# NVlabs/motion-policy-networks

Hardware: AMD Instinct MI355X
Metric: env-steps/sec (FK+SDF+PointNet++) (higher is better)
Workload: dtype f32

## Files before the change

include/mpinets_hip.h:

```cpp
#ifndef MPINETS_HIP_H
#define MPINETS_HIP_H

#include <stdint.h>

#ifdef __cplusplus
extern "C" {
#endif

typedef void *mpx_stream_t;

#define MPX_NUM_FRAMES 15

int mpx_version(void);
const char *mpx_last_error(void);
int mpx_device_info(char *name, int name_len, int *cu_count, int *lds_bytes);


int mpx_prim_frames(const float *centers, const float *quats, int n, float *inv_frames,
                    mpx_stream_t stream);

int mpx_cuboid_sdf(const float *inv_frames, const float *dims, int B, int M, const float *points,
                   int P, float *out, mpx_stream_t stream);
int mpx_cylinder_sdf(const float *inv_frames, const float *radii, const float *heights, int B,
                     int M, const float *points, int P, float *out, mpx_stream_t stream);
// ... 137 lines not shown

int mpx_scene_cloud(const float *cub_centers, const float *cub_dims, const float *cub_quats, int M1,
                    const float *cyl_centers, const float *cyl_radii, const float *cyl_heights,
                    const float *cyl_quats, int M2, int B, int num_points, uint64_t seed,
                    int64_t env_offset, uint16_t *assign, uint8_t *labels, int32_t *n_obstacles, float *out,
                    int64_t out_batch_stride, int out_point_stride, int write_label,
                    mpx_stream_t stream);


int mpx_fps(const float *xyz, int B, int N, int stride, int npoint, int32_t *idx, float *new_xyz,
            int new_stride, mpx_stream_t stream);

#define MPX_VARIANT_FPS 0
#define MPX_VARIANT_BALL_QUERY 1
#define MPX_VARIANT_UNIT_QUEUE 2
#define MPX_VARIANT_COUNT_ 3
int mpx_set_variant(int what, int value);
int mpx_get_variant(int what);

int mpx_ball_query(const float *new_xyz, int new_stride, const float *xyz, int stride, int B,
                   int N, int npoint, float radius, int nsample, int32_t *idx, int32_t *cnt,
                   mpx_stream_t stream);

int mpx_ball_query_hits(const float *new_xyz, int new_stride, const float *xyz, int stride, int B,
                        int N, int npoint, float radius, int nsample, int32_t *idx, int32_t *cnt,
                        mpx_stream_t stream);

int mpx_sort_queries(const int32_t *cnt, int64_t n, int nsample, int32_t *order, int32_t *scratch,
                     mpx_stream_t stream);

int mpx_group_points(const float *xyz, int stride, const float *new_xyz, int new_stride,
                     const float *feat, int feat_stride, int C, const int32_t *idx, int B, int N,
                     int npoint, int nsample, float *out, mpx_stream_t stream);

int mpx_sa_mlp(const float *xyz, int stride, const float *new_xyz, int new_stride,
               const float *feat, int feat_stride, int C, const int32_t *idx, const int32_t *cnt,
               int B, int N, int npoint, int nsample, const float *wpack, int c1, int c2, int c3,
               float *out, int out_stride, int append_centre, mpx_stream_t stream);
int mpx_sa_mlp_factored(const float *pre, const float *ctr, const int32_t *idx, const int32_t *cnt, int B,
                        int N, int npoint, int nsample, const float *wpack, int C, int c1, int c2, int c3,
                        float *out, int out_stride, mpx_stream_t stream);
int mpx_sa_mlp_bf16x3_factored_wants_order(void);
int mpx_sa_mlp_bf16x3_factored(const float *pre, const float *ctr, const int32_t *idx, const int32_t *cnt,
                               const int32_t *order, int B, int N, int npoint, int nsample, const void *wpack,
                               int C, int c1, int c2, int c3, float *out, int out_stride, mpx_stream_t stream);
int64_t mpx_sa_pack_size(int C, int c1, int c2, int c3);
int mpx_sa_pack_weights(const float *w1, const float *b1, const float *w2, const float *b2,
                        const float *w3, const float *b3, int C, int c1, int c2, int c3,
                        float *wpack, mpx_stream_t stream);

int mpx_sa_mlp_bf16x3_wants_order(int C, int c1, int c2, int c3, int nsample);
int mpx_sa_mlp_bf16x3(const float *xyz, int stride, const float *new_xyz, int new_stride,
                      const float *feat, int feat_stride, int C, const int32_t *idx,
                      const int32_t *cnt, const int32_t *order, int B, int N, int npoint,
                      int nsample, const void *wpack, int c1, int c2, int c3, float *out,
                      int out_stride, int append_centre, mpx_stream_t stream);
// ... 106 lines not shown
```

motion-policy-networks_amd/csrc/common.h:

```cpp
#pragma once
#include <hip/hip_runtime.h>

#include <atomic>
#include <type_traits>
#include <stdint.h>
#include <stdio.h>

#include "../../include/mpinets_hip.h"

#define MPX_EXPORT extern "C" __attribute__((visibility("default")))

void mpx_set_error(const char *fmt, ...);

#define MPX_REQUIRE(cond, ...)        \
  do {                                \
    if (!(cond)) {                    \
      mpx_set_error(__VA_ARGS__);     \
      return 1;                       \
    }                                 \
  } while (0)

#define MPX_LDS_LIMIT_ONCE(kernel, bytes, what)                                                                \
  do {                                                                                                         \
    static std::atomic<unsigned long long> lds_done_{0};                                                       \
// ... 10 lines not shown

#define MPX_LAUNCH_CHECK(name)                                              \
  do {                                                                      \
    hipError_t e_ = hipGetLastError();                                      \
    if (e_ != hipSuccess) {                                                 \
      mpx_set_error("%s: launch failed: %s", name, hipGetErrorString(e_)); \
      return 2;                                                             \
    }                                                                       \
    return 0;                                                               \
  } while (0)

static inline hipStream_t mpx_s(mpx_stream_t s) { return reinterpret_cast<hipStream_t>(s); }
unsigned int *mpx_unit_queue_for(hipStream_t stream, int *exhausted);
int mpx_unit_queue_slots();
void mpx_unit_queue_set_slots(int n);
static inline int cdiv(int64_t a, int64_t b) { return (int)((a + b - 1) / b); }

int mpx_segmax_check(const char *name, int M, const int32_t *seg, int64_t Q, int N, const void *keys, const float *pooled,
                     int ldp, const int64_t *arg);
int mpx_segmax_unpack_launch(const unsigned long long *keys, int64_t Q, int N, float *pooled, int ldp, int64_t *arg,
                             hipStream_t stream);
void mpx_wgrad_bf16x3_launch(const float *dy, int lddy, const float *x, int ldx, int M, int N, int K, int rows_per_split,
                             int S, float *partial, int with_bias, hipStream_t stream);
void mpx_reduce_partials_launch(const float *partial, int S, int64_t stride, int64_t n, float *out, hipStream_t stream);

constexpr int MPX_GRID_Y = 65535;
static inline int64_t mpx_row_slab(int bm, int64_t row_bytes) {
  int64_t blocks = 65528;
  if (row_bytes > 0) {
    const int64_t fit = ((((int64_t)1 << 32) - 8192) / row_bytes / bm) & ~(int64_t)7;
// ... 206 lines not shown
```

motion-policy-networks_amd/csrc/pointnet.hip:

```cpp
#include "common.h"

#include <stdlib.h>
#include <type_traits>

typedef unsigned long long u64;

template <int CTRL>
__device__ __forceinline__ u64 dpp_mov64(u64 v) {
  unsigned lo = (unsigned)v, hi = (unsigned)(v >> 32);
  lo = (unsigned)__builtin_amdgcn_update_dpp(0, (int)lo, CTRL, 0xf, 0xf, true);
  hi = (unsigned)__builtin_amdgcn_update_dpp(0, (int)hi, CTRL, 0xf, 0xf, true);
  return ((u64)hi << 32) | lo;
}
struct U32Pair {
  unsigned lo, hi;
};
__device__ __forceinline__ u64 pack64(unsigned lo, unsigned hi) { return __builtin_bit_cast(u64, U32Pair{lo, hi}); }
__device__ __forceinline__ u64 umax64(u64 a, u64 b) {
  double r;
  asm("v_max_f64 %0, %1, %2" : "=v"(r) : "v"(__builtin_bit_cast(double, a)), "v"(__builtin_bit_cast(double, b)));
  return __builtin_bit_cast(u64, r);
}

__device__ __forceinline__ u64 row_max64(u64 v) {
// ... 509 lines not shown
  }
}

#ifndef MPX_FPS4_MIN_B
#define MPX_FPS4_MIN_B 768
#endif
constexpr int FPS_MAX_N = 8192;
constexpr int FPS_MAX_LDS = 256 + 3 * FPS_MAX_N * 4;

static int opt_n_threads_log2(int n) {
  int l = 0;
  while ((2 << l) <= n && (2 << l) <= 512) ++l;
  return l;
}

static std::atomic<int> g_variant[MPX_VARIANT_COUNT_] = {{1}, {1}, {1}};
MPX_EXPORT int mpx_set_variant(int what, int value) {
  MPX_REQUIRE(what >= 0 && what < MPX_VARIANT_COUNT_, "mpx_set_variant: unknown selector %d", what);
  MPX_REQUIRE(value == 0 || value == 1, "mpx_set_variant: value must be 0 (plain kernels) or 1 (default)");
  g_variant[what].store(value, std::memory_order_relaxed);
  if (what == MPX_VARIANT_UNIT_QUEUE) mpx_unit_queue_set_slots(value ? 256 : 0);
  return 0;
}
MPX_EXPORT int mpx_get_variant(int what) {
  return (what >= 0 && what < MPX_VARIANT_COUNT_) ? g_variant[what].load(std::memory_order_relaxed) : -1;
}

MPX_EXPORT int mpx_fps(const float *xyz, int B, int N, int stride, int npoint, int32_t *idx, float *new_xyz,
                       int new_stride, mpx_stream_t stream) {
  MPX_REQUIRE(B >= 0 && N >= 1 && npoint >= 0 && stride >= 3, "mpx_fps: bad size");
  MPX_REQUIRE(N <= FPS_MAX_N, "mpx_fps: N = %d > %d unsupported", N, FPS_MAX_N);
// ... 627 lines not shown
```

motion-policy-networks_amd/csrc/sa_mlp.hip:

```cpp
#include "common.h"

#include <stdlib.h>
#include <type_traits>

typedef float f32x16 __attribute__((ext_vector_type(16)));

#define PAD_CH (-1)
constexpr int SA_MAX_NSAMPLE = 256;
#ifndef MPX_SA1_Q
#define MPX_SA1_Q 32
#endif
#ifndef MPX_SA2_Q
#define MPX_SA2_Q 8
#endif
#ifndef MPX_SA1_GR
#define MPX_SA1_GR 2
#endif
#ifndef MPX_SA_SPREAD
#define MPX_SA_SPREAD 1
#endif
#ifndef MPX_SA1_LDSPOOL
#define MPX_SA1_LDSPOOL 1
#endif

template <int CF, int C1, int C2, int C3>
struct SaCfg {
  static_assert(CF == 1 || CF % 2 == 0, "feature channels must be 1 or even");
  static_assert(C1 % 32 == 0 && C2 % 32 == 0 && C3 % 32 == 0, "layer widths must be multiples of 32");
  static constexpr int CIN = 3 + CF;
  static constexpr int KS0 = (CF == 1) ? 2 : 2 + CF / 2;
  static constexpr int KS1 = C1 / 2, KS2 = C2 / 2;
  static constexpr int OT1 = C1 / 32, OT2 = C2 / 32, OT3 = C3 / 32;
// ... 202 lines not shown
    }
  }

  float *orow = out + qid * out_stride;
#pragma unroll
  for (int ot = 0; ot < Cfg::OT3; ++ot) {
    float v = omax[ot];
    v = mpx_max_across_halves(v);
    const int ch = ot * 32 + col;
    v = fmaxf(v + bias3[ch], 0.0f);
    if (half == 0) orow[ch] = v;
  }
}


template <int CF, int C1, int C2, int C3, int Q, bool FACT, int MAXNS = SA_MAX_NSAMPLE>
__global__ void __launch_bounds__(64) __attribute__((amdgpu_waves_per_eu(CF == 1 ? 4 : 2, CF == 1 ? 4 : 2)))
    sa_mlp_packed_kernel(const float *__restrict__ xyz, int stride, const float *__restrict__ new_xyz,
                         int new_stride, const float *__restrict__ feat, int feat_stride,
                         const int32_t *__restrict__ idx, const int32_t *__restrict__ cnt, int64_t n_query, int N,
                         int npoint, int nsample, const float *__restrict__ wpack, float *__restrict__ out,
                         int out_stride, int bpe, const float *__restrict__ pre_rows, const float *__restrict__ ctr,
                         int append_centre, unsigned int *__restrict__ queue) {
  using Cfg = SaCfg<CF, C1, C2, C3>;
  constexpr int GR = CF == 1 ? MPX_SA1_GR : 4, NGRP = 32 / GR;
  static_assert(GR == 2 || GR == 4, "pooling groups of 2 or 4 rows");
  __shared__ float ctr_s[FACT ? Q * C1 : 1];
  constexpr bool LPOOL = CF == 1 && !FACT && MPX_SA1_LDSPOOL != 0 && MAXNS <= 128;
  __shared__ __attribute__((aligned(16))) float pool_s[LPOOL ? Q * C3 : 1];
  __shared__ __attribute__((aligned(16))) unsigned char qmap_s[Q * MAXNS / GR + 32];
  __shared__ __attribute__((aligned(16))) float b1_s[C1], b2_s[C2], b3_s[C3];
  static_assert(Q >= 1 && Q <= 32, "queries per wave");
  const int lane = threadIdx.x & 63;
  const int half = lane >> 5, col = lane & 31;
  const int64_t n_units = (n_query + Q - 1) / Q;
  const int xcd = blockIdx.x & 7;
  const int64_t j_end = bpe > 0 ? n_units / 8 : n_units;
  int steal = 0;
  auto next_unit = [&]() __attribute__((always_inline)) {
    unsigned int v = 0;
    if (lane == 0) v = atomicAdd(queue + (bpe > 0 ? ((xcd + steal) & 7) : 0), 1u);
    return (int64_t)(unsigned int)__builtin_amdgcn_readfirstlane((int)v);
  };
  const __amdgpu_buffer_rsrc_t wrsrc =
      __builtin_amdgcn_make_buffer_rsrc(const_cast<float *>(wpack), 0, (int)(Cfg::TOTAL * 4), 0x00020000);
  const int wvoff = lane * 16;
  for (int i = threadIdx.x; i < C1; i += 64) b1_s[i] = wpack[Cfg::B1_OFF + i];
  for (int i = threadIdx.x; i < C2; i += 64) b2_s[i] = wpack[Cfg::B2_OFF + i];
  for (int i = threadIdx.x; i < C3; i += 64) b3_s[i] = wpack[Cfg::B3_OFF + i];
  constexpr int G1 = FACT ? 0 : Cfg::S1 / 4, G2 = Cfg::S2 / 4, G3 = Cfg::S3 / 4, GT = G1 + G2 + G3;
  constexpr bool LAZY = FACT && MPX_SA_SPREAD;
  constexpr int CH = 4, NC0 = (GT + CH - 1) / CH, NC = NC0 + (NC0 & 1);
// ... 8 lines not shown
    int wb = (int)(FACT ? Cfg::W2_OFF : Cfg::W1_OFF) * 4;
    asm volatile("" : "+s"(wb));
    fetch(0, wb);
  }
  int64_t j_next = queue ? next_unit() : 0;
  for (bool first = true;; first = false) {
  int64_t wg;
  if (queue) {
    int64_t j = j_next;
    bool dry = false;
    while (j >= j_end) {
      if (bpe == 0 || ++steal == 8) {
        dry = true;
        break;
      }
      j = next_unit();
    }
    if (dry) break;
    wg = bpe > 0 ? ((j / bpe) * 8 + ((xcd + steal) & 7)) * bpe + j % bpe : j;
  } else {
    if (!first) break;
    wg = blockIdx.x;
    if (bpe > 0) {
      const int64_t slot = wg >> 3;
      wg = ((slot / bpe) * 8 + xcd) * bpe + slot % bpe;
    }
  }
  const int64_t q0 = wg * Q;
  const int nq = (int)min((int64_t)Q, n_query - q0);
  if constexpr (LPOOL) {
    const float ninf = -__builtin_inff();
#pragma unroll
    for (int e = lane; e < Q * C3 / 4; e += 64) *reinterpret_cast<float4 *>(pool_s + 4 * e) = make_float4(ninf, ninf, ninf, ninf);
  }
  if constexpr (FACT) {
#pragma unroll
    for (int i = threadIdx.x; i < Q * C1 / 4; i += 64) {
      const int qi = (4 * i) / C1;
      if (qi < nq)
        *reinterpret_cast<float4 *>(ctr_s + 4 * i) = *reinterpret_cast<const float4 *>(ctr + q0 * C1 + 4 * i);
    }
    __syncthreads();
  }

  int my_cnt = 0, my_rows = 0;
  if (lane < nq) {
    const int c = cnt[q0 + lane];
    my_cnt = c <= 0 ? 1 : (c > nsample ? nsample : c);
// ... 296 lines not shown
            __builtin_amdgcn_sched_group_barrier(0x020, 1, 0);
          }
        } else {
#pragma unroll
          for (int u = 0; u < CH; ++u) {
            __builtin_amdgcn_sched_group_barrier(0x008, 4, 0);
            __builtin_amdgcn_sched_group_barrier(0x020, 1, 0);
          }
        }
      }
    }
    if constexpr (!LPOOL) cur = gq(NGRP - 1);
  }
  if constexpr (LPOOL) {
#pragma unroll 2
    for (int e = lane; e < Q * C3 / 4; e += 64) {
      const int qi = (4 * e) / C3, ch = (4 * e) % C3;
      if (qi < nq) {
        const float4 v = *reinterpret_cast<const float4 *>(pool_s + 4 * e), bb = *reinterpret_cast<const float4 *>(b3_s + ch);
        *reinterpret_cast<float4 *>(out + (int64_t)(qbase + qi) * out_stride + ch) =
            make_float4(fmaxf(v.x + bb.x, 0.0f), fmaxf(v.y + bb.y, 0.0f), fmaxf(v.z + bb.z, 0.0f), fmaxf(v.w + bb.w, 0.0f));
      }
    }
  } else {
#pragma unroll
    for (int ot = 0; ot < Cfg::OT3; ++ot) flush(ot, cur);
  }
  }
}

static int64_t sa_wave_slots(int per_cu) {
  static std::atomic<int> cus[64];
  int dev = 0;
  if (hipGetDevice(&dev) != hipSuccess) return 0;
  int n = cus[dev & 63].load(std::memory_order_relaxed);
  if (n == 0) {
    if (hipDeviceGetAttribute(&n, hipDeviceAttributeMultiprocessorCount, dev) != hipSuccess || n <= 0) return 0;
    cus[dev & 63].store(n, std::memory_order_relaxed);
  }
  return ((int64_t)n * per_cu) & ~(int64_t)7;
}
template <int CF, int C1, int C2, int C3>
static int launch_sa(const float *xyz, int stride, const float *new_xyz, int new_stride, const float *feat,
                     int feat_stride, const int32_t *idx, const int32_t *cnt, int B, int N, int npoint, int nsample,
                     const float *wpack, float *out, int out_stride, int append_centre, mpx_stream_t stream) {
  const int64_t nq = (int64_t)B * npoint;
  MPX_REQUIRE(nq / 4 + 1 < ((int64_t)1 << 31), "mpx_sa_mlp: too many query points");
  MPX_REQUIRE(!append_centre || (cnt && out_stride >= C3 + 4),
              "mpx_sa_mlp: append_centre needs the hit counts and out_stride >= c3 + 4");
  MPX_REQUIRE(!append_centre || nsample <= SA_MAX_NSAMPLE, "mpx_sa_mlp: append_centre needs nsample <= %d", SA_MAX_NSAMPLE);
  if (cnt && nsample <= SA_MAX_NSAMPLE) {
    constexpr int QL = CF == 1 ? MPX_SA1_Q : 8, QS = CF == 1 ? 4 : 2;
    int rc = 0;
    auto go = [&](auto qtag) {
      constexpr int Q = decltype(qtag)::value;
      int64_t nw = (nq + Q - 1) / Q;
// ... 1 lines not shown
      unsigned int *queue = nullptr;
      const int64_t slots = sa_wave_slots(CF == 1 ? 16 : 8);
      if (slots > 0 && nw >= 4 * slots) {
        int exhausted = 0;
        queue = mpx_unit_queue_for(mpx_s(stream), &exhausted);
        if (!queue && !exhausted) {
          mpx_set_error("mpx_sa_mlp: cannot reset the unit queue");
          rc = 1;
          return;
        }
        if (queue) nw = slots;
      }
      bool lpool = false;
      if constexpr (CF == 1 && MPX_SA1_LDSPOOL != 0) {
        lpool = nsample <= 128 && out_stride % 4 == 0 && ((uintptr_t)out & 15) == 0;
        if (lpool)
          hipLaunchKernelGGL((sa_mlp_packed_kernel<CF, C1, C2, C3, Q, false, 128>), dim3((unsigned)nw), dim3(64), 0,
                             mpx_s(stream), xyz, stride, new_xyz, new_stride, feat, feat_stride, idx, cnt, nq, N, npoint,
                             nsample, wpack, out, out_stride, bpe, nullptr, nullptr, append_centre, queue);
      }
      if (!lpool)
        hipLaunchKernelGGL((sa_mlp_packed_kernel<CF, C1, C2, C3, Q, false>), dim3((unsigned)nw), dim3(64), 0,
                           mpx_s(stream), xyz, stride, new_xyz, new_stride, feat, feat_stride, idx, cnt, nq, N, npoint,
                           nsample, wpack, out, out_stride, bpe, nullptr, nullptr, append_centre, queue);
    };
    if (nq >= 1024 * QL) go(std::integral_constant<int, QL>{});
    else go(std::integral_constant<int, QS>{});
    if (rc) return rc;
  } else {
    hipLaunchKernelGGL((sa_mlp_kernel<CF, C1, C2, C3>), dim3((unsigned)((nq + 3) / 4)), dim3(256), 0,
// ... 47 lines not shown
    constexpr int Q = decltype(qtag)::value;
    int64_t nw = (nq + Q - 1) / Q;
    const int bpe = (npoint % Q == 0 && B % 8 == 0) ? npoint / Q : 0;
    unsigned int *queue = nullptr;
    const int64_t slots = sa_wave_slots(8);
    if (slots > 0 && nw >= 4 * slots) {
      int exhausted = 0;
      queue = mpx_unit_queue_for(mpx_s(stream), &exhausted);
      if (!queue && !exhausted) {
        mpx_set_error("mpx_sa_mlp_factored: cannot reset the unit queue");
        rc = 1;
        return;
      }
      if (queue) nw = slots;
    }
    hipLaunchKernelGGL((sa_mlp_packed_kernel<64, 128, 128, 256, Q, true>), dim3((unsigned)nw), dim3(64), 0,
                       mpx_s(stream), nullptr, 0, nullptr, 0, nullptr, 0, idx, cnt, nq, N, npoint, nsample, wpack, out,
                       out_stride, bpe, pre, ctr, 0, queue);
  };
  if (nq >= 1024 * MPX_SA2_Q) go(std::integral_constant<int, MPX_SA2_Q>{});
  else if (nq >= 1024) go(std::integral_constant<int, 2>{});
  else go(std::integral_constant<int, 1>{});
  if (rc) return rc;
  MPX_LAUNCH_CHECK("mpx_sa_mlp_factored");
}

MPX_EXPORT int64_t mpx_sa_pack_size(int C, int c1, int c2, int c3) {
#define CALL(a, b, c, d) return SaCfg<a, b, c, d>::TOTAL
  if (C == 1 && c1 == 64 && c2 == 64 && c3 == 64) { CALL(1, 64, 64, 64); }
  else if (C == 64 && c1 == 128 && c2 == 128 && c3 == 256) { CALL(64, 128, 128, 256); }
// ... 21 lines not shown
```

motion-policy-networks_amd/mpinets_amd/_lib.py:

```python
from __future__ import annotations

import ctypes
import os
from ctypes import c_char_p, c_float, c_int, c_int64, c_void_p
from typing import Optional

import torch

_HERE = os.path.dirname(os.path.abspath(__file__))
LIB_PATH = os.environ.get("MPX_LIB_PATH") or os.path.join(_HERE, "libmpinets_hip.so")

P, I, F, L = c_void_p, c_int, c_float, c_int64

PROTOTYPES = {
    "mpx_version": [],
    "mpx_device_info": [c_char_p, I, P, P],
    "mpx_prim_frames": [P, P, I, P, P],
    "mpx_cuboid_sdf": [P, P, I, I, P, I, P, P],
    "mpx_cylinder_sdf": [P, P, P, I, I, P, I, P, P],
    "mpx_sphere_sdf": [P, P, I, I, P, I, P, P],
    "mpx_franka_fk": [P, I, F, P, P],
    "mpx_franka_cloud": [P, I, F, P, P, P, I, P, L, I, P],
    "mpx_pose_cloud": [P, I, P, P, I, P, L, I, P],
    "mpx_franka_spheres": [P, I, F, P, P, I, P, P],
# ... 19 lines not shown
    "mpx_pool_dgrad": [P, I, P, P, I, P, L, I, I, P, I, P, I, I, I, I, P, I, P],
    "mpx_batch_configs": [P, L, I, P, P, P, F, ctypes.c_uint64, L, I, I, F, P, P, P, P, P, P],
    "mpx_gather_rows": [P, P, I, I, P, P],
    "mpx_depth_render": [P, F, F, F, F, I, I, I, P, P, I, P, P, P, I, P, P, I, F, P, P],
    "mpx_depth_select": [P, P, F, F, F, F, I, I, I, I, ctypes.c_uint64, L, P, L, I, P, P],
    "mpx_scene_cloud": [P, P, P, I, P, P, P, P, I, I, I, ctypes.c_uint64, L, P, P, P, P, L, I, I, P],
    "mpx_set_variant": [I, I],
    "mpx_get_variant": [I],
    "mpx_fps": [P, I, I, I, I, P, P, I, P],
    "mpx_ball_query": [P, I, P, I, I, I, I, F, I, P, P, P],
    "mpx_ball_query_hits": [P, I, P, I, I, I, I, F, I, P, P, P],
    "mpx_sort_queries": [P, L, I, P, P, P],
    "mpx_group_points": [P, I, P, I, P, I, I, P, I, I, I, I, P, P],
    "mpx_sa_mlp": [P, I, P, I, P, I, I, P, P, I, I, I, I, P, I, I, I, P, I, I, P],
    "mpx_sa_mlp_factored": [P, P, P, P, I, I, I, I, P, I, I, I, I, P, I, P],
    "mpx_sa_mlp_bf16x3_factored_wants_order": [],
    "mpx_sa_mlp_bf16x3_factored": [P, P, P, P, P, I, I, I, I, P, I, I, I, I, P, I, P],
    "mpx_sa_pack_size": [I, I, I, I],
    "mpx_sa_pack_weights": [P, P, P, P, P, P, I, I, I, I, P, P],
    "mpx_sa_mlp_bf16x3": [P, I, P, I, P, I, I, P, P, P, I, I, I, I, P, I, I, I, P, I, I, P],
    "mpx_sa_mlp_bf16x3_wants_order": [I, I, I, I, I],
    "mpx_sa_pack_bf16x3_size": [I, I, I, I],
    "mpx_sa_pack_bf16x3": [P, P, P, P, P, P, I, I, I, I, P, P],
    "mpx_sa3_pack_size": [I, I, I, I],
    "mpx_sa3_pack_weights": [P, I, P, P, P, P, P, I, I, I, I, P, P],
    "mpx_sa3_chain": [P, I, I, I, P, I, I, I, I, P, I, P],
    "mpx_sa3_chain_probe": [P, I, I, P, P, I, P, P],
    "mpx_sa2_bf16x3_set_probe": [P],
    "mpx_linear": [P, I, P, P, I, I, I, I, P, I, P],
    "mpx_linear_workspace": [I, I, I],
# ... 15 lines not shown
    "mpx_linear_dact": [P, I, P, I, I, I, P, I, I, P, I, P],
    "mpx_linear_bf16x3_dact": [P, I, P, I, I, I, P, I, I, P, I, P],
    "mpx_linear_wgrad_bf16x3": [P, I, P, I, I, I, I, P, P, P, P],
    "mpx_linear_wgrad_scratch": [I, I, I],
    "mpx_linear_wgrad": [P, I, P, I, I, I, I, P, P, P, P],
    "mpx_groupnorm_leaky": [P, P, P, I, I, I, F, P, P],
    "mpx_groupnorm_leaky_to_pairs": [P, P, P, I, I, I, F, P, I, P],
    "mpx_rowmax": [P, I, I, I, I, P, I, P],
    "mpx_append_columns": [P, I, I, I, L, P, I, I, P],
    "mpx_policy_workspace": [I, I],
    "mpx_policy_forward": [P, P, I, P, I, P, P, L, P],
    "mpx_rollout_workspace": [I, I],
    "mpx_rollout_step": [P, P, P, I, P, P, I, P, P, P, L, P],
    "mpx_rollout": [P, P, P, P, I, P, P, I, P, P, P, L, P],
}
RESTYPES = {"mpx_last_error": c_char_p, "mpx_sa_pack_size": c_int64, "mpx_sa3_front_bf16x3_pack_size": c_int64, "mpx_sa_pack_bf16x3_size": c_int64,
            "mpx_linear_wgrad_scratch": c_int64, "mpx_pool_wgrad_scratch": c_int64, "mpx_linear_workspace": c_int64, "mpx_policy_workspace": c_int64, "mpx_rollout_workspace": c_int64}

_lib: Optional[ctypes.CDLL] = None


class MpxError(RuntimeError):
    pass


def load() -> ctypes.CDLL:
    global _lib
    if _lib is not None:
        return _lib
    if not os.path.exists(LIB_PATH):
        raise MpxError(
# ... 93 lines not shown
```

motion-policy-networks_amd/mpinets_amd/pointnet2.py:

```python
from __future__ import annotations

from typing import Any, Callable, List, Optional, Tuple

import torch
from torch import nn

from . import _lib


def furthest_point_sample(xyz: torch.Tensor, npoint: int, return_xyz: bool = False):
    _lib.require_cuda(xyz)
    assert xyz.ndim == 3 and xyz.size(2) >= 3 and xyz.dtype == torch.float32 and xyz.is_contiguous()
    B, N, S = xyz.shape
    idx = torch.empty((B, npoint), dtype=torch.int32, device=xyz.device)
    new_xyz = torch.empty((B, npoint, 3), dtype=torch.float32, device=xyz.device) if return_xyz else None
    _lib.call("mpx_fps", _lib.ptr(xyz), B, N, S, npoint, _lib.ptr(idx), _lib.ptr(new_xyz), 3)
    return (idx, new_xyz) if return_xyz else idx


def gather_operation(features: torch.Tensor, idx: torch.Tensor) -> torch.Tensor:
    return torch.gather(features, 2, idx.long().unsqueeze(1).expand(-1, features.size(1), -1))


def ball_query(radius: float, nsample: int, xyz: torch.Tensor, new_xyz: torch.Tensor, return_counts: bool = False):
# ... 32 lines not shown
    need = _lib.load().mpx_linear_workspace(M, N, K)
    if need == 0:
        _lib.call("mpx_linear", _lib.ptr(x), x.stride(0), _lib.ptr(weight), _lib.ptr(bias), M, N, K, act,
                  _lib.ptr(out), out.stride(0))
    else:
        key = (x.device, _lib.stream_ptr())
        ws = _WORKSPACE.get(key)
        if ws is None or ws.numel() < need:
            ws = _WORKSPACE[key] = torch.empty(max(need, 16 << 20), dtype=torch.uint8, device=x.device)
        _lib.call("mpx_linear_ws", _lib.ptr(x), x.stride(0), _lib.ptr(weight), _lib.ptr(bias), M, N, K, act,
                  _lib.ptr(out), out.stride(0), _lib.ptr(ws), ws.numel())
    return out


_WORKSPACE = {}


def split_pairs(x: torch.Tensor, out: Optional[torch.Tensor] = None) -> torch.Tensor:
    assert x.ndim == 2 and x.stride(1) == 1 and x.dtype == torch.float32
    R, K = x.shape
    Kp = (K + 15) // 16 * 16
    if out is None:
        out = torch.empty((R, 2 * Kp), dtype=torch.bfloat16, device=x.device)
    assert out.shape == (R, 2 * Kp) and out.stride(1) == 1
    _lib.call("mpx_split_bf16", _lib.ptr(x), x.stride(0), R, K, _lib.ptr(out), out.stride(0))
    return out


class DerivedWeights:

# ... 86 lines not shown
                raise _lib.MpxError(f"unsupported shared-MLP shape C={C} mlp=({c1},{c2},{c3})")
            _lib.call(fn, _lib.ptr(w[0]), _lib.ptr(b[0]), _lib.ptr(w[1]), _lib.ptr(b[1]), _lib.ptr(w[2]),
                      _lib.ptr(b[2]), C, c1, c2, c3, _lib.ptr(pack))
            return pack

        return self.entry(("pack", precision), [p for c in convs for p in (c.weight, c.bias)], make)


def launch_sa(precision: str, xyz_ptr: int, stride: int, new_xyz_ptr: int, new_stride: int, feat_ptr: int,
              feat_stride: int, C: int, idx: torch.Tensor, cnt: Optional[torch.Tensor], B: int, N: int, npoint: int,
              nsample: int, wpack: torch.Tensor, widths: Tuple[int, int, int], out_ptr: int, out_stride: int,
              append_centre: bool = False) -> bool:
    c1, c2, c3 = widths
    if precision == "fp32":
        fused = bool(append_centre and cnt is not None)
        _lib.call("mpx_sa_mlp", xyz_ptr, stride, new_xyz_ptr, new_stride, feat_ptr, feat_stride, C, _lib.ptr(idx),
                  _lib.ptr(cnt), B, N, npoint, nsample, _lib.ptr(wpack), c1, c2, c3, out_ptr, out_stride, int(fused))
        return fused
    order = None
    wants_order = bool(_lib.load().mpx_sa_mlp_bf16x3_wants_order(C, c1, c2, c3, nsample))
    if cnt is not None and wants_order:
        order = torch.empty(B * npoint, dtype=torch.int32, device=idx.device)
        scratch = torch.empty(128, dtype=torch.int32, device=idx.device)
        _lib.call("mpx_sort_queries", _lib.ptr(cnt), B * npoint, nsample, _lib.ptr(order), _lib.ptr(scratch))
    fused = bool(append_centre and not wants_order)
    _lib.call("mpx_sa_mlp_bf16x3", xyz_ptr, stride, new_xyz_ptr, new_stride, feat_ptr, feat_stride, C, _lib.ptr(idx),
              _lib.ptr(cnt), _lib.ptr(order), B, N, npoint, nsample, _lib.ptr(wpack), c1, c2, c3, out_ptr, out_stride,
              int(fused))
    return fused

# ... 11 lines not shown
    launch_sa(precision, _lib.ptr(xyz), S, _lib.ptr(new_xyz), new_xyz.stride(1), _lib.ptr(feat), feat_stride, C, idx, cnt,
              B, N, npoint, nsample, wpack, widths, _lib.ptr(out), out.stride(1))
    return out


def sa_mlp_factored(point_rows: torch.Tensor, centre_rows: torch.Tensor, idx: torch.Tensor, cnt: torch.Tensor,
                    packed: SAWeights, convs: List[nn.Conv2d], C: int, N: int, out_ptr: int, out_stride: int,
                    precision: str = "fp32") -> None:
    B, npoint, nsample = idx.shape
    wp, wc, nb1 = packed.factored(convs, C)
    c1, c2, c3 = (c.out_channels for c in convs)
    pre = linear(point_rows, wp, None)
    ctr = linear(centre_rows, wc, nb1)
    x3 = precision == "bf16x3"
    order = (None,) if x3 else ()
    _lib.call("mpx_sa_mlp_bf16x3_factored" if x3 else "mpx_sa_mlp_factored", _lib.ptr(pre), _lib.ptr(ctr), _lib.ptr(idx),
              _lib.ptr(cnt), *order, B, N, npoint, nsample, _lib.ptr(packed.get(convs, C, precision)), C, c1, c2, c3, out_ptr,
              out_stride)


FACTORED_SHAPE = (64, 128, 128, 256)
FACTORED_BF16X3_MAX_NSAMPLE = 128


def use_factored(module: "PointnetSAModule", C: int, convs) -> bool:
    if not module.factored or (C,) + tuple(c.out_channels for c in convs) != FACTORED_SHAPE:
        return False
    return module.precision != "bf16x3" or module.nsample <= FACTORED_BF16X3_MAX_NSAMPLE


# ... 393 lines not shown
```

Measured before the change: 97950.

## Cut SA MLP work into variable-length query units balanced by neighbour rows

Adds a pre-pass that reads per-query neighbour counts, computes per-environment prefix sums, and cuts queries into variable-length units capped by total sample rows (near a nominal query count), then packs them into per-XCD queues. The fp32 SA MLP kernels (module 1 LDS-pool path and the factored module 2 path) consume these units instead of fixed Q-query chunks. The aim is to even out per-wave work when neighbourhood sizes vary and avoid padding to nsample. It costs two extra small kernel launches per SA call, a device workspace registered per stream, larger Q templates and possible LDS/register pressure changes.

```diff
diff --git a/include/mpinets_hip.h b/include/mpinets_hip.h
--- a/include/mpinets_hip.h
+++ b/include/mpinets_hip.h
@@ -175,7 +175,8 @@
 #define MPX_VARIANT_FPS 0
 #define MPX_VARIANT_BALL_QUERY 1
 #define MPX_VARIANT_UNIT_QUEUE 2
-#define MPX_VARIANT_COUNT_ 3
+#define MPX_VARIANT_UNIT_CUT 3
+#define MPX_VARIANT_COUNT_ 4
 int mpx_set_variant(int what, int value);
 int mpx_get_variant(int what);
 
@@ -201,6 +202,11 @@
 int mpx_sa_mlp_factored(const float *pre, const float *ctr, const int32_t *idx, const int32_t *cnt, int B,
                         int N, int npoint, int nsample, const float *wpack, int C, int c1, int c2, int c3,
                         float *out, int out_stride, mpx_stream_t stream);
+int64_t mpx_sa_unit_workspace(int C, int B, int npoint, int nsample);
+int mpx_sa_set_unit_workspace(void *workspace, int64_t workspace_bytes, mpx_stream_t stream);
+int mpx_sa_unit_tiles(int C, int64_t *tiles, int64_t *units, mpx_stream_t stream);
+int mpx_sa_unit_cut(int C, const int32_t *cnt, int B, int npoint, int nsample, void *workspace, int64_t workspace_bytes,
+                    int64_t *layout, mpx_stream_t stream);
 int mpx_sa_mlp_bf16x3_factored_wants_order(void);
 int mpx_sa_mlp_bf16x3_factored(const float *pre, const float *ctr, const int32_t *idx, const int32_t *cnt,
                                const int32_t *order, int B, int N, int npoint, int nsample, const void *wpack,
diff --git a/motion-policy-networks_amd/csrc/common.h b/motion-policy-networks_amd/csrc/common.h
--- a/motion-policy-networks_amd/csrc/common.h
+++ b/motion-policy-networks_amd/csrc/common.h
@@ -48,6 +48,7 @@
 unsigned int *mpx_unit_queue_for(hipStream_t stream, int *exhausted);
 int mpx_unit_queue_slots();
 void mpx_unit_queue_set_slots(int n);
+int mpx_variant_value(int what);
 static inline int cdiv(int64_t a, int64_t b) { return (int)((a + b - 1) / b); }
 
 int mpx_segmax_check(const char *name, int M, const int32_t *seg, int64_t Q, int N, const void *keys, const float *pooled,
diff --git a/motion-policy-networks_amd/csrc/pointnet.hip b/motion-policy-networks_amd/csrc/pointnet.hip
--- a/motion-policy-networks_amd/csrc/pointnet.hip
+++ b/motion-policy-networks_amd/csrc/pointnet.hip
@@ -547,7 +547,8 @@
   return l;
 }
 
-static std::atomic<int> g_variant[MPX_VARIANT_COUNT_] = {{1}, {1}, {1}};
+static std::atomic<int> g_variant[MPX_VARIANT_COUNT_] = {{1}, {1}, {1}, {1}};
+int mpx_variant_value(int what) { return g_variant[what].load(std::memory_order_relaxed); }
 MPX_EXPORT int mpx_set_variant(int what, int value) {
   MPX_REQUIRE(what >= 0 && what < MPX_VARIANT_COUNT_, "mpx_set_variant: unknown selector %d", what);
   MPX_REQUIRE(value == 0 || value == 1, "mpx_set_variant: value must be 0 (plain kernels) or 1 (default)");
diff --git a/motion-policy-networks_amd/csrc/sa_mlp.hip b/motion-policy-networks_amd/csrc/sa_mlp.hip
--- a/motion-policy-networks_amd/csrc/sa_mlp.hip
+++ b/motion-policy-networks_amd/csrc/sa_mlp.hip
@@ -1,7 +1,9 @@
 #include "common.h"
 
 #include <stdlib.h>
+#include <mutex>
 #include <type_traits>
+#include <unordered_map>
 
 typedef float f32x16 __attribute__((ext_vector_type(16)));
 
@@ -16,6 +18,10 @@
 #ifndef MPX_SA1_GR
 #define MPX_SA1_GR 2
 #endif
+constexpr int SA1_QMIN = 24, SA1_QMAX = 36, SA1_UROWS = 2048;
+constexpr int SA2_QMIN = 6, SA2_QMAX = 10, SA2_UROWS = 1024;
+static_assert(SA1_QMIN <= MPX_SA1_Q && MPX_SA1_Q <= SA1_QMAX && SA2_QMIN <= MPX_SA2_Q && MPX_SA2_Q <= SA2_QMAX, "nominal unit length");
+constexpr int SA_UNIT_MAX_NPOINT = 1024;
 #ifndef MPX_SA_SPREAD
 #define MPX_SA_SPREAD 1
 #endif
@@ -248,28 +254,32 @@
 }
 
 
-template <int CF, int C1, int C2, int C3, int Q, bool FACT, int MAXNS = SA_MAX_NSAMPLE>
+template <int CF, int C1, int C2, int C3, int Q, bool FACT, int MAXNS = SA_MAX_NSAMPLE, int UROWS = 0>
 __global__ void __launch_bounds__(64) __attribute__((amdgpu_waves_per_eu(CF == 1 ? 4 : 2, CF == 1 ? 4 : 2)))
     sa_mlp_packed_kernel(const float *__restrict__ xyz, int stride, const float *__restrict__ new_xyz,
                          int new_stride, const float *__restrict__ feat, int feat_stride,
                          const int32_t *__restrict__ idx, const int32_t *__restrict__ cnt, int64_t n_query, int N,
                          int npoint, int nsample, const float *__restrict__ wpack, float *__restrict__ out,
                          int out_stride, int bpe, const float *__restrict__ pre_rows, const float *__restrict__ ctr,
-                         int append_centre, unsigned int *__restrict__ queue) {
+                         int append_centre, unsigned int *__restrict__ queue, const int2 *__restrict__ units = nullptr,
+                         const unsigned int *__restrict__ ucount = nullptr, int64_t qstride = 0) {
   using Cfg = SaCfg<CF, C1, C2, C3>;
+  constexpr bool VAR = UROWS > 0;
   constexpr int GR = CF == 1 ? MPX_SA1_GR : 4, NGRP = 32 / GR;
   static_assert(GR == 2 || GR == 4, "pooling groups of 2 or 4 rows");
   __shared__ float ctr_s[FACT ? Q * C1 : 1];
   constexpr bool LPOOL = CF == 1 && !FACT && MPX_SA1_LDSPOOL != 0 && MAXNS <= 128;
   __shared__ __attribute__((aligned(16))) float pool_s[LPOOL ? Q * C3 : 1];
-  __shared__ __attribute__((aligned(16))) unsigned char qmap_s[Q * MAXNS / GR + 32];
+  __shared__ __attribute__((aligned(16))) unsigned char qmap_s[(VAR ? UROWS : Q * MAXNS) / GR + 32];
   __shared__ __attribute__((aligned(16))) float b1_s[C1], b2_s[C2], b3_s[C3];
-  static_assert(Q >= 1 && Q <= 32, "queries per wave");
+  static_assert(Q >= 1 && Q <= (VAR ? 64 : 32), "queries per wave");
+  static_assert(!VAR || UROWS >= MAXNS, "a unit holds at least one whole neighbourhood");
   const int lane = threadIdx.x & 63;
   const int half = lane >> 5, col = lane & 31;
   const int64_t n_units = (n_query + Q - 1) / Q;
   const int xcd = blockIdx.x & 7;
-  const int64_t j_end = bpe > 0 ? n_units / 8 : n_units;
+  int64_t j_end = bpe > 0 ? n_units / 8 : n_units;
+  if constexpr (VAR) j_end = ucount[bpe > 0 ? xcd : 0];
   int steal = 0;
   auto next_unit = [&]() __attribute__((always_inline)) {
     unsigned int v = 0;
@@ -308,10 +318,12 @@
         dry = true;
         break;
       }
+      if constexpr (VAR) j_end = ucount[(xcd + steal) & 7];
       j = next_unit();
     }
     if (dry) break;
-    wg = bpe > 0 ? ((j / bpe) * 8 + ((xcd + steal) & 7)) * bpe + j % bpe : j;
+    if constexpr (VAR) wg = (bpe > 0 ? ((xcd + steal) & 7) * qstride : 0) + j;
+    else wg = bpe > 0 ? ((j / bpe) * 8 + ((xcd + steal) & 7)) * bpe + j % bpe : j;
   } else {
     if (!first) break;
     wg = blockIdx.x;
@@ -320,12 +332,18 @@
       wg = ((slot / bpe) * 8 + xcd) * bpe + slot % bpe;
     }
   }
-  const int64_t q0 = wg * Q;
-  const int nq = (int)min((int64_t)Q, n_query - q0);
+  int64_t q0 = wg * Q;
+  int nq = (int)min((int64_t)Q, n_query - q0);
+  if constexpr (VAR) {
+    const int2 u = units[wg];
+    q0 = u.x;
+    nq = u.y;
+  }
+  const int qlim = VAR ? nq : Q;
   if constexpr (LPOOL) {
     const float ninf = -__builtin_inff();
 #pragma unroll
-    for (int e = lane; e < Q * C3 / 4; e += 64) *reinterpret_cast<float4 *>(pool_s + 4 * e) = make_float4(ninf, ninf, ninf, ninf);
+    for (int e = lane; e < qlim * C3 / 4; e += 64) *reinterpret_cast<float4 *>(pool_s + 4 * e) = make_float4(ninf, ninf, ninf, ninf);
   }
   if constexpr (FACT) {
 #pragma unroll
@@ -652,7 +670,7 @@
   }
   if constexpr (LPOOL) {
 #pragma unroll 2
-    for (int e = lane; e < Q * C3 / 4; e += 64) {
+    for (int e = lane; e < qlim * C3 / 4; e += 64) {
       const int qi = (4 * e) / C3, ch = (4 * e) % C3;
       if (qi < nq) {
         const float4 v = *reinterpret_cast<const float4 *>(pool_s + 4 * e), bb = *reinterpret_cast<const float4 *>(b3_s + ch);
@@ -678,6 +696,254 @@
   }
   return ((int64_t)n * per_cu) & ~(int64_t)7;
 }
+__global__ void __launch_bounds__(64)
+    sa_unit_cut_kernel(const int32_t *__restrict__ cnt, int npoint, int nsample, int gr, int qmin, int qnom, int qmax,
+                       int cap, int upe, int2 *__restrict__ tmp, unsigned int *__restrict__ nun,
+                       unsigned int *__restrict__ til) {
+  __shared__ int pre_s[SA_UNIT_MAX_NPOINT + 1];
+  const int lane = threadIdx.x;
+  const int64_t env = blockIdx.x;
+  int carry = 0;
+  if (lane == 0) pre_s[0] = 0;
+  for (int i0 = 0; i0 < npoint; i0 += 64) {
+    const int i = i0 + lane;
+    int r = 0;
+    if (i < npoint) {
+      const int c = cnt[env * npoint + i];
+      const int cc = c <= 0 ? 1 : (c > nsample ? nsample : c);
+      r = (cc + gr - 1) / gr * gr;
+    }
+#pragma unroll
+    for (int o = 1; o < 64; o <<= 1) {
+      const int t = __shfl_up(r, o);
+      if (lane >= o) r += t;
+    }
+    if (i < npoint) pre_s[i + 1] = carry + r;
+    carry += __shfl(r, 63);
+  }
+  __syncthreads();
+  int s = 0, u = 0;
+  unsigned int tiles = 0;
+  while (s < npoint) {
+    const int rem = npoint - s, lo = min(qmin, rem), hi = min(qmax, rem), base = pre_s[s];
+    const int L = lo + lane;
+    int key = 0x7fffffff;
+    if (L <= hi) {
+      const int rows = pre_s[s + L] - base;
+      const int d = L > qnom ? L - qnom : qnom - L;
+      if (rows <= cap) key = ((-rows & 31) << 16) | (d << 8) | L;
+    }
+#pragma unroll
+    for (int o = 32; o >= 1; o >>= 1) key = min(key, __shfl_xor(key, o));
+    int len;
+    if (key != 0x7fffffff) {
+      len = key & 0xff;
+    } else {
+      int l = 0;
+      if (1 + lane < lo && pre_s[s + 1 + lane] - base <= cap) l = 1 + lane;
+#pragma unroll
+      for (int o = 32; o >= 1; o >>= 1) l = max(l, __shfl_xor(l, o));
+      len = max(l, 1);
+    }
+    tiles += (unsigned int)((pre_s[s + len] - base + 31) >> 5);
+    if (lane == 0 && u < upe) tmp[env * upe + u] = make_int2((int)(env * npoint + s), len);
+    ++u;
+    s += len;
+  }
+  if (lane == 0) {
+    nun[env] = (unsigned int)min(u, upe);
+    til[env] = tiles;
+  }
+}
+
+constexpr int SA_UNIT_COPY_WGS = 16;
+__global__ void __launch_bounds__(256)
+    sa_unit_queue_kernel(const int2 *__restrict__ tmp, const unsigned int *__restrict__ nun,
+                         const unsigned int *__restrict__ til, int B, int nq, int upe, int64_t qstride,
+                         int2 *__restrict__ units, unsigned int *__restrict__ hdr) {
+  __shared__ unsigned int wsum_s[2][4];
+  const int tid = threadIdx.x, lane = tid & 63, wave = tid >> 6;
+  const int x = blockIdx.y, sh = blockIdx.x;
+  const int n_env = (B - x + nq - 1) / nq;
+  unsigned int base = 0, tiles = 0;
+  for (int c = 0; c * 256 < n_env; ++c) {
+    const int i = c * 256 + tid;
+    const int64_t e = x + (int64_t)nq * i;
+    const unsigned int n = i < n_env ? nun[e] : 0u;
+    unsigned int incl = n, t = i < n_env ? til[e] : 0u;
+#pragma unroll
+    for (int o = 1; o < 64; o <<= 1) {
+      const unsigned int v = __shfl_up(incl, o);
+      if (lane >= o) incl += v;
+    }
+#pragma unroll
+    for (int o = 32; o >= 1; o >>= 1) t += __shfl_xor(t, o);
+    __syncthreads();
+    if (lane == 63) {
+      wsum_s[0][wave] = incl;
+      wsum_s[1][wave] = t;
+    }
+    __syncthreads();
+    unsigned int off = base + incl - n;
+    for (int w = 0; w < 4; ++w) {
+      if (w < wave) off += wsum_s[0][w];
+      base += wsum_s[0][w];
+      tiles += wsum_s[1][w];
+    }
+    if ((c * 4 + wave) % SA_UNIT_COPY_WGS == sh) {
+      const int2 *src = tmp + e * upe;
+      int2 *dst = units + x * qstride + off;
+#pragma unroll 4
+      for (unsigned int k = 0; k < n; ++k) dst[k] = src[k];
+    }
+  }
+  if (sh == 0 && tid == 0) {
+    hdr[x] = base;
+    hdr[8 + x] = tiles;
+  }
+  if (sh == 0 && x == 0 && tid >= nq && tid < 8) hdr[tid] = hdr[8 + tid] = 0;
+}
+
+static int64_t sa_units_per_env(int npoint, int nsample, int gr, int qmin, int cap) {
+  const int64_t nsr = (nsample + gr - 1) / gr * gr;
+  return npoint / qmin + 1 + (int64_t)npoint * nsr / (cap - nsr + 1);
+}
+static int64_t pad256(int64_t n) { return (n + 255) / 256 * 256; }
+
+struct SaUnitPlan {
+  int nq, upe;
+  int64_t qstride, bytes;
+  unsigned int *hdr, *nun, *til;
+  int2 *tmp, *units;
+};
+static SaUnitPlan sa_unit_plan(char *base, int module, int B, int npoint, int nsample) {
+  SaUnitPlan p;
+  const int gr = module == 0 ? MPX_SA1_GR : 4;
+  p.nq = B % 8 == 0 ? 8 : 1;
+  p.upe = (int)sa_units_per_env(npoint, nsample, gr, module == 0 ? SA1_QMIN : SA2_QMIN, module == 0 ? SA1_UROWS : SA2_UROWS);
+  p.qstride = (int64_t)((B + p.nq - 1) / p.nq) * p.upe;
+  int64_t used = 256;
+  auto take = [&](int64_t n) {
+    char *q = base ? base + used : nullptr;
+    used += pad256(n);
+    return q;
+  };
+  p.hdr = reinterpret_cast<unsigned int *>(base) + 32 * module;
+  p.nun = reinterpret_cast<unsigned int *>(take((int64_t)B * 4));
+  p.til = reinterpret_cast<unsigned int *>(take((int64_t)B * 4));
+  p.tmp = reinterpret_cast<int2 *>(take((int64_t)B * p.upe * 8));
+  p.units = reinterpret_cast<int2 *>(take(p.qstride * p.nq * 8));
+  p.bytes = used;
+  return p;
+}
+
+struct SaUnitWs {
+  void *ptr;
+  int64_t bytes;
+};
+static std::mutex sa_unit_ws_mu;
+static std::unordered_map<unsigned long long, SaUnitWs> sa_unit_ws;
+static unsigned long long sa_stream_key(mpx_stream_t stream) {
+  int dev = 0;
+  (void)hipGetDevice(&dev);
+  return ((unsigned long long)(dev & 63) << 56) ^ (unsigned long long)(uintptr_t)stream;
+}
+static SaUnitWs sa_unit_ws_of(mpx_stream_t stream) {
+  std::lock_guard<std::mutex> lock(sa_unit_ws_mu);
+  auto it = sa_unit_ws.find(sa_stream_key(stream));
+  return it == sa_unit_ws.end() ? SaUnitWs{nullptr, 0} : it->second;
+}
+static bool sa_units_eligible(int module, int B, int npoint, int nsample) {
+  const int64_t nq = (int64_t)B * npoint;
+  const int64_t slots = sa_wave_slots(module == 0 ? 16 : 8);
+  const int Q = module == 0 ? MPX_SA1_Q : MPX_SA2_Q;
+  return nq >= 1024 * Q && slots > 0 && (nq + Q - 1) / Q >= 4 * slots && npoint <= SA_UNIT_MAX_NPOINT &&
+         nsample <= (module == 0 ? 128 : SA_MAX_NSAMPLE);
+}
+
+MPX_EXPORT int64_t mpx_sa_unit_workspace(int C, int B, int npoint, int nsample) {
+  if (B <= 0 || npoint <= 0 || nsample <= 0 || (C != 1 && C != 64)) return 0;
+  const int module = C == 1 ? 0 : 1;
+  if (!sa_units_eligible(module, B, npoint, nsample)) return 0;
+  return sa_unit_plan(nullptr, module, B, npoint, nsample).bytes;
+}
+
+MPX_EXPORT int mpx_sa_set_unit_workspace(void *workspace, int64_t workspace_bytes, mpx_stream_t stream) {
+  MPX_REQUIRE(workspace == nullptr || (((uintptr_t)workspace & 255) == 0 && workspace_bytes >= 256),
+              "mpx_sa_set_unit_workspace: the workspace must be 256-byte aligned and hold at least 256 bytes");
+  std::lock_guard<std::mutex> lock(sa_unit_ws_mu);
+  if (workspace) {
+    if (hipMemsetAsync(workspace, 0, 256, mpx_s(stream)) != hipSuccess) {
+      mpx_set_error("mpx_sa_set_unit_workspace: cannot clear the workspace header");
+      return 1;
+    }
+    sa_unit_ws[sa_stream_key(stream)] = SaUnitWs{workspace, workspace_bytes};
+  } else {
+    sa_unit_ws.erase(sa_stream_key(stream));
+  }
+  return 0;
+}
+
+MPX_EXPORT int mpx_sa_unit_tiles(int C, int64_t *tiles, int64_t *units, mpx_stream_t stream) {
+  MPX_REQUIRE(C == 1 || C == 64, "mpx_sa_unit_tiles: C selects the module, 1 or 64");
+  MPX_REQUIRE(tiles && units, "mpx_sa_unit_tiles: NULL result pointer");
+  const SaUnitWs ws = sa_unit_ws_of(stream);
+  MPX_REQUIRE(ws.ptr, "mpx_sa_unit_tiles: no unit workspace is registered for this stream");
+  unsigned int h[16];
+  hipError_t e = hipMemcpyAsync(h, static_cast<unsigned int *>(ws.ptr) + (C == 1 ? 0 : 32), sizeof(h), hipMemcpyDeviceToHost,
+                                mpx_s(stream));
+  if (e == hipSuccess) e = hipStreamSynchronize(mpx_s(stream));
+  MPX_REQUIRE(e == hipSuccess, "mpx_sa_unit_tiles: %s", hipGetErrorString(e));
+  *tiles = *units = 0;
+  for (int x = 0; x < 8; ++x) {
+    *units += h[x];
+    *tiles += h[8 + x];
+  }
+  return 0;
+}
+
+static void sa_launch_cut(int module, const int32_t *cnt, int B, int npoint, int nsample, mpx_stream_t stream, const SaUnitPlan &p);
+static bool sa_cut_units(int module, const int32_t *cnt, int B, int npoint, int nsample, mpx_stream_t stream, SaUnitPlan &p) {
+  if (!mpx_variant_value(MPX_VARIANT_UNIT_CUT) || !sa_units_eligible(module, B, npoint, nsample)) return false;
+  const SaUnitWs ws = sa_unit_ws_of(stream);
+  if (!ws.ptr) return false;
+  p = sa_unit_plan(static_cast<char *>(ws.ptr), module, B, npoint, nsample);
+  if (p.bytes > ws.bytes) return false;
+  sa_launch_cut(module, cnt, B, npoint, nsample, stream, p);
+  return true;
+}
+static void sa_launch_cut(int module, const int32_t *cnt, int B, int npoint, int nsample, mpx_stream_t stream, const SaUnitPlan &p) {
+  const int gr = module == 0 ? MPX_SA1_GR : 4;
+  if (module == 0)
+    hipLaunchKernelGGL(sa_unit_cut_kernel, dim3((unsigned)B), dim3(64), 0, mpx_s(stream), cnt, npoint, nsample, gr, SA1_QMIN,
+                       MPX_SA1_Q, SA1_QMAX, SA1_UROWS, p.upe, p.tmp, p.nun, p.til);
+  else
+    hipLaunchKernelGGL(sa_unit_cut_kernel, dim3((unsigned)B), dim3(64), 0, mpx_s(stream), cnt, npoint, nsample, gr, SA2_QMIN,
+                       MPX_SA2_Q, SA2_QMAX, SA2_UROWS, p.upe, p.tmp, p.nun, p.til);
+  hipLaunchKernelGGL(sa_unit_queue_kernel, dim3(SA_UNIT_COPY_WGS, p.nq), dim3(256), 0, mpx_s(stream), p.tmp, p.nun, p.til, B,
+                     p.nq, p.upe, p.qstride, p.units, p.hdr);
+}
+
+MPX_EXPORT int mpx_sa_unit_cut(int C, const int32_t *cnt, int B, int npoint, int nsample, void *workspace,
+                               int64_t workspace_bytes, int64_t *layout, mpx_stream_t stream) {
+  MPX_REQUIRE(C == 1 || C == 64, "mpx_sa_unit_cut: C selects the module, 1 or 64");
+  MPX_REQUIRE(cnt && layout && B >= 1 && npoint >= 1 && npoint <= SA_UNIT_MAX_NPOINT && nsample >= 1 &&
+                  nsample <= (C == 1 ? 128 : SA_MAX_NSAMPLE) && (int64_t)B * npoint < ((int64_t)1 << 31),
+              "mpx_sa_unit_cut: bad size (npoint <= %d, nsample <= %d)", SA_UNIT_MAX_NPOINT, C == 1 ? 128 : SA_MAX_NSAMPLE);
+  MPX_REQUIRE(workspace && ((uintptr_t)workspace & 255) == 0, "mpx_sa_unit_cut: the workspace must be 256-byte aligned");
+  const int module = C == 1 ? 0 : 1;
+  const SaUnitPlan p = sa_unit_plan(static_cast<char *>(workspace), module, B, npoint, nsample);
+  layout[0] = p.nq;
+  layout[1] = p.qstride;
+  layout[2] = reinterpret_cast<char *>(p.units) - static_cast<char *>(workspace);
+  layout[3] = reinterpret_cast<char *>(p.hdr) - static_cast<char *>(workspace);
+  layout[4] = p.bytes;
+  MPX_REQUIRE(workspace_bytes >= p.bytes, "mpx_sa_unit_cut: workspace of %lld bytes, %lld needed", (long long)workspace_bytes,
+              (long long)p.bytes);
+  sa_launch_cut(module, cnt, B, npoint, nsample, stream, p);
+  MPX_LAUNCH_CHECK("mpx_sa_unit_cut");
+}
+
 template <int CF, int C1, int C2, int C3>
 static int launch_sa(const float *xyz, int stride, const float *new_xyz, int new_stride, const float *feat,
                      int feat_stride, const int32_t *idx, const int32_t *cnt, int B, int N, int npoint, int nsample,
@@ -709,6 +975,16 @@
       bool lpool = false;
       if constexpr (CF == 1 && MPX_SA1_LDSPOOL != 0) {
         lpool = nsample <= 128 && out_stride % 4 == 0 && ((uintptr_t)out & 15) == 0;
+        if constexpr (Q == QL) {
+          SaUnitPlan up;
+          if (lpool && queue && sa_cut_units(0, cnt, B, npoint, nsample, stream, up)) {
+            hipLaunchKernelGGL((sa_mlp_packed_kernel<CF, C1, C2, C3, SA1_QMAX, false, 128, SA1_UROWS>), dim3((unsigned)nw), dim3(64),
+                               0, mpx_s(stream), xyz, stride, new_xyz, new_stride, feat, feat_stride, idx, cnt, nq, N, npoint,
+                               nsample, wpack, out, out_stride, up.nq == 8 ? 1 : 0, nullptr, nullptr, append_centre, queue,
+                               up.units, up.hdr, up.qstride);
+            return;
+          }
+        }
         if (lpool)
           hipLaunchKernelGGL((sa_mlp_packed_kernel<CF, C1, C2, C3, Q, false, 128>), dim3((unsigned)nw), dim3(64), 0,
                              mpx_s(stream), xyz, stride, new_xyz, new_stride, feat, feat_stride, idx, cnt, nq, N, npoint,
@@ -786,6 +1062,15 @@
       }
       if (queue) nw = slots;
     }
+    if constexpr (Q == MPX_SA2_Q) {
+      SaUnitPlan up;
+      if (queue && sa_cut_units(1, cnt, B, npoint, nsample, stream, up)) {
+        hipLaunchKernelGGL((sa_mlp_packed_kernel<64, 128, 128, 256, SA2_QMAX, true, SA_MAX_NSAMPLE, SA2_UROWS>), dim3((unsigned)nw),
+                           dim3(64), 0, mpx_s(stream), nullptr, 0, nullptr, 0, nullptr, 0, idx, cnt, nq, N, npoint, nsample,
+                           wpack, out, out_stride, up.nq == 8 ? 1 : 0, pre, ctr, 0, queue, up.units, up.hdr, up.qstride);
+        return;
+      }
+    }
     hipLaunchKernelGGL((sa_mlp_packed_kernel<64, 128, 128, 256, Q, true>), dim3((unsigned)nw), dim3(64), 0,
                        mpx_s(stream), nullptr, 0, nullptr, 0, nullptr, 0, idx, cnt, nq, N, npoint, nsample, wpack, out,
                        out_stride, bpe, pre, ctr, 0, queue);
diff --git a/motion-policy-networks_amd/mpinets_amd/_lib.py b/motion-policy-networks_amd/mpinets_amd/_lib.py
--- a/motion-policy-networks_amd/mpinets_amd/_lib.py
+++ b/motion-policy-networks_amd/mpinets_amd/_lib.py
@@ -57,6 +57,10 @@
     "mpx_group_points": [P, I, P, I, P, I, I, P, I, I, I, I, P, P],
     "mpx_sa_mlp": [P, I, P, I, P, I, I, P, P, I, I, I, I, P, I, I, I, P, I, I, P],
     "mpx_sa_mlp_factored": [P, P, P, P, I, I, I, I, P, I, I, I, I, P, I, P],
+    "mpx_sa_unit_workspace": [I, I, I, I],
+    "mpx_sa_set_unit_workspace": [P, L, P],
+    "mpx_sa_unit_tiles": [I, P, P, P],
+    "mpx_sa_unit_cut": [I, P, I, I, I, P, L, P, P],
     "mpx_sa_mlp_bf16x3_factored_wants_order": [],
     "mpx_sa_mlp_bf16x3_factored": [P, P, P, P, P, I, I, I, I, P, I, I, I, I, P, I, P],
     "mpx_sa_pack_size": [I, I, I, I],
@@ -102,7 +106,7 @@
     "mpx_rollout_step": [P, P, P, I, P, P, I, P, P, P, L, P],
     "mpx_rollout": [P, P, P, P, I, P, P, I, P, P, P, L, P],
 }
-RESTYPES = {"mpx_last_error": c_char_p, "mpx_sa_pack_size": c_int64, "mpx_sa3_front_bf16x3_pack_size": c_int64, "mpx_sa_pack_bf16x3_size": c_int64,
+RESTYPES = {"mpx_last_error": c_char_p, "mpx_sa_unit_workspace": c_int64, "mpx_sa_pack_size": c_int64, "mpx_sa3_front_bf16x3_pack_size": c_int64, "mpx_sa_pack_bf16x3_size": c_int64,
             "mpx_linear_wgrad_scratch": c_int64, "mpx_pool_wgrad_scratch": c_int64, "mpx_linear_workspace": c_int64, "mpx_policy_workspace": c_int64, "mpx_rollout_workspace": c_int64}
 
 _lib: Optional[ctypes.CDLL] = None
diff --git a/motion-policy-networks_amd/mpinets_amd/pointnet2.py b/motion-policy-networks_amd/mpinets_amd/pointnet2.py
--- a/motion-policy-networks_amd/mpinets_amd/pointnet2.py
+++ b/motion-policy-networks_amd/mpinets_amd/pointnet2.py
@@ -70,6 +70,36 @@
 
 
 _WORKSPACE = {}
+_UNIT_WS = {}
+_UNIT_WS_NEED = {}
+
+
+def ensure_unit_workspace(C: int, B: int, npoint: int, nsample: int, device) -> None:
+    shape = (C, B, npoint, nsample)
+    need = _UNIT_WS_NEED.get(shape)
+    if need is None:
+        need = _UNIT_WS_NEED[shape] = int(_lib.load().mpx_sa_unit_workspace(C, B, npoint, nsample))
+    if need == 0:
+        return
+    key = (device, _lib.stream_ptr())
+    ws = _UNIT_WS.get(key)
+    if ws is None or ws.numel() < need:
+        ws = _UNIT_WS[key] = torch.empty(need, dtype=torch.uint8, device=device)
+        _lib.call("mpx_sa_set_unit_workspace", _lib.ptr(ws), ws.numel())
+
+
+def unit_tiles(C: int):
+    import ctypes
+
+    t, u = ctypes.c_int64(0), ctypes.c_int64(0)
+    _lib.call("mpx_sa_unit_tiles", C, ctypes.addressof(t), ctypes.addressof(u))
+    return int(t.value), int(u.value)
+
+
+def set_unit_cut(on: bool) -> None:
+    lib = _lib.load()
+    if lib.mpx_set_variant(3, int(bool(on))) != 0:
+        raise _lib.MpxError(lib.mpx_last_error().decode())
 
 
 def split_pairs(x: torch.Tensor, out: Optional[torch.Tensor] = None) -> torch.Tensor:
@@ -186,6 +216,8 @@
     c1, c2, c3 = widths
     if precision == "fp32":
         fused = bool(append_centre and cnt is not None)
+        if cnt is not None:
+            ensure_unit_workspace(C, B, npoint, nsample, idx.device)
         _lib.call("mpx_sa_mlp", xyz_ptr, stride, new_xyz_ptr, new_stride, feat_ptr, feat_stride, C, _lib.ptr(idx),
                   _lib.ptr(cnt), B, N, npoint, nsample, _lib.ptr(wpack), c1, c2, c3, out_ptr, out_stride, int(fused))
         return fused
@@ -227,6 +259,8 @@
     ctr = linear(centre_rows, wc, nb1)
     x3 = precision == "bf16x3"
     order = (None,) if x3 else ()
+    if not x3:
+        ensure_unit_workspace(C, B, npoint, nsample, idx.device)
     _lib.call("mpx_sa_mlp_bf16x3_factored" if x3 else "mpx_sa_mlp_factored", _lib.ptr(pre), _lib.ptr(ctr), _lib.ptr(idx),
               _lib.ptr(cnt), *order, B, N, npoint, nsample, _lib.ptr(packed.get(convs, C, precision)), C, c1, c2, c3, out_ptr,
               out_stride)
```

New measurement: 98850, median of 6. Within noise of the previous version (+0.9%).
